# DiligentGraphics/DiligentFX

Measured on AMD Instinct MI355X. Metric: Mpixels/s full PBR+postFX chain @4K; %HBM roofline; 1/2/4/8-GPU scaling, higher is better.
Workload: dtype f32; 1 GPU; full chain PBR+SSR+SSAO+composite+TAA+Bloom+ToneMap 3840x2160 per GPU (BASELINE configs[3]); width=3840, height_per_gpu=2160, storage=fp32 planes, taa=bicubic, ssao=GTAO full-res, ssr=full-res rays, tonemap=Uncharted2+sRGB, ibl=static maps: the shade's apron copy is made once (mifx_postfx_set_static_ibl), fusion_mask=31

## Files before the change

### diligentfx_amd/csrc/api_bloom_taa.cpp

```cpp
#include <cmath>

#include "mifx_objects.h"

using namespace mifx;

mifx_bloom::~mifx_bloom()
{
    for (auto* p : down) delete p;
    for (auto* p : up) delete p;
}

static uint32_t compute_mip_levels_count(uint32_t w, uint32_t h)
{
    uint32_t m = w > h ? w : h, n = 0;
    while (m > 0) { ++n; m >>= 1; }
    return n;
}

extern "C" {

mifx_status mifx_bloom_create(mifx_postfx* ctx, mifx_bloom** out)
{
    MIFX_REQUIRE(ctx != nullptr && out != nullptr, "mifx_bloom_create: null argument");
    *out        = new mifx_bloom();
// ... 59 lines not shown
    p.taa = rows_finer(p.compute0, 4, H);
    const int last = mipCount - 1;
    for (int i = G > 0 ? G : 1; i <= last; ++i) p.up[i] = rows_coarser(p.up[i - 1], 3, int(up[i]->h));
    if (G == 0) p.up[0] = rows_coarser(need, 3, int(up[0]->h));
    p.down[last] = p.up[last];
    for (int i = last - 1; i > G; --i) p.down[i] = rows_hull(p.up[i], rows_finer(p.down[i + 1], 4, int(down[i]->h)));
    return p;
}

mifx_status mifx_bloom::run(const mifx_bloom_render_attribs* ra, int phase, const FusedToneMap* tone_map, const Request& req)
{
    MIFX_RANGE("Bloom");
    mifx_postfx* c = ra->postfx ? ra->postfx : ctx;
    Img  color;
    bool packed = false;
    MIFX_CHECK(to_img_hdr(ra->color, "color", color, packed));
    MIFX_REQUIRE(uint32_t(color.w) == w && uint32_t(color.h) == h, "mifx_bloom_execute: color is %dx%d, the effect was prepared for %ux%u", color.w, color.h, w, h);
    const mifx_bloom_attribs& a = *ra->attribs;
    const int mipCount = mip_count(a);
    MIFX_REQUIRE(mipCount >= 2 && mipCount <= int(down.size()),
                 "mifx_bloom_execute: Radius %g gives %d pyramid levels; the reference reads an unwritten texture below 2 levels", a.Radius, mipCount);
    MIFX_HIP_CHECK(hipSetDevice(c->device));
    hipStream_t s = c->stream;
    const Rows need = c->needed_rows(int(h));
    const Plan p    = make_plan(c->band, need, mipCount, req.halo_level0);
    MIFX_REQUIRE(phase == 0 || p.G >= 0, "mifx_bloom_execute: phased execution needs a row band (mifx_chain_set_row_band)");
    MIFX_REQUIRE(phase != 0 || p.G < 0, "mifx_bloom_execute: a row band is set; run the two phases around the gather of down[%d]", p.G);
    auto dwin = [&](int i) { return p.G >= 0 ? win(down[i]->view(), p.down[i]) : down[i]->view(); };
    auto uwin = [&](int i) { return p.G >= 0 ? win(up[i]->view(), p.up[i]) : up[i]->view(); };
    const int last = mipCount - 1;
    int first = mipCount;
    for (int i = 1; i < mipCount; ++i)
        if (down[i]->w * down[i]->h <= kTailTexels) { first = i; break; }
    bool tail = p.G < 0 && fuse_tail && last >= first + 1 && last - first + 2 <= 8;
    Img  tailDown[8], tailUp[8];
    if (tail)
    {
        for (int i = first - 1; i <= last; ++i) { tailDown[i - first + 1] = down[i]->view(); tailUp[i - first + 1] = up[i]->view(); }
        tail = bloom_tail_fits(tailDown, last - first + 2);
    }
    const int  wide = tail ? first : mipCount;
    if (phase != 2)
    {
        {
            MifxKernelTimer timer(c, "bloom_prefilter_kernel");
            MIFX_CHECK(launch_bloom_prefilter(s, color, p.G >= 0 ? win(down[0]->view(), p.compute0) : down[0]->view(), a, packed));
        }
        if (p.G >= 0 && req.after_level0) MIFX_CHECK(req.after_level0(*down[0], s));
        for (int i = 1; i < wide && (p.G < 0 || i <= p.G); ++i) MIFX_CHECK(launch_bloom_downsample(s, down[i - 1]->view(), dwin(i)));
        if (phase == 1) return MIFX_OK;
    }
    if (p.G >= 0)
        for (int i = p.G + 1; i < wide; ++i) MIFX_CHECK(launch_bloom_downsample(s, down[i - 1]->view(), dwin(i)));
    if (tail) MIFX_CHECK(launch_bloom_tail(s, tailDown, tailUp, last - first + 2));
    for (int i = tail ? first : last; i > 0; --i)
        MIFX_CHECK(launch_bloom_upsample(s, down[i - 1]->view(), i != last ? up[i]->view() : down[i]->view(), uwin(i - 1), a, false));
    if (tone_map)
    {
        MIFX_REQUIRE(tone_map->attribs->iToneMappingMode >= 0 && tone_map->attribs->iToneMappingMode <= MIFX_TONE_MAPPING_MODE_COMMERCE, "unknown tone mapping mode %d",
                     tone_map->attribs->iToneMappingMode);
        MIFX_REQUIRE((tone_map->flags & ~uint32_t(MIFX_TONEMAP_FLAG_CONVERT_OUTPUT_TO_SRGB)) == 0, "unknown tone map flags 0x%x", tone_map->flags);
        Img ldr;
        MIFX_CHECK(to_img_wh(tone_map->ldr, MIFX_FORMAT_F32X4, w, h, "ldr_out", ldr));
        MifxKernelTimer timer(c, "bloom_upsample_tonemap_kernel");
        MIFX_CHECK(launch_bloom_final_tonemap(s, color, up[0]->view(), win(output.view(), need), ldr, a, *tone_map->attribs, tone_map->ave_log_lum, tone_map->flags, !tone_map->skip_output, packed));
        output_deferred  = tone_map->skip_output;
        deferred_color   = color;
        deferred_packed  = packed;
        deferred_attribs = a;
        deferred_rows    = need;
    }
    else
    {
        MifxKernelTimer timer(c, "bloom_upsample_kernel");
        MIFX_CHECK(launch_bloom_upsample(s, color, up[0]->view(), win(output.view(), need), a, true, packed));
        output_deferred = false;
    }
    return MIFX_OK;
}

mifx_status mifx_bloom::run_deferred_output()
{
    if (!output_deferred) return MIFX_OK;
    MIFX_HIP_CHECK(hipSetDevice(ctx->device));
    ctx->queued_outside_execute();
    MIFX_CHECK(launch_bloom_upsample(ctx->stream, deferred_color, up[0]->view(), win(output.view(), deferred_rows), deferred_attribs, true, deferred_packed));
    output_deferred = false;
    return MIFX_OK;
}

mifx_status mifx_bloom_execute(mifx_bloom* fx, const mifx_bloom_render_attribs* ra)
{
    MIFX_REQUIRE(fx != nullptr && ra != nullptr && ra->attribs != nullptr, "mifx_bloom_execute: null argument");
    if (!fx->prepared)
    {
        set_error("mifx_bloom_execute: mifx_bloom_prepare must be called first");
        return MIFX_ERR_INVALID_OP;
    }
    return fx->run(ra, 0, nullptr, mifx_bloom::Request{});
}

mifx_status mifx_bloom_get_output(mifx_bloom* fx, mifx_image2d* out)
{
    MIFX_REQUIRE(fx != nullptr && out != nullptr, "mifx_bloom_get_output: null argument");
    if (!fx->prepared)
    {
        set_error("mifx_bloom_get_output: resources are not prepared");
        return MIFX_ERR_INVALID_OP;
    }
    MIFX_CHECK(fx->run_deferred_output());
    *out = fx->output.desc();
    return MIFX_OK;
}

mifx_status mifx_debug_bloom_set_tail(mifx_bloom* fx, int32_t enable)
{
    MIFX_REQUIRE(fx != nullptr, "mifx_debug_bloom_set_tail: null argument");
    fx->fuse_tail = enable != 0;
    return MIFX_OK;
}

mifx_status mifx_bloom_get_intermediate(mifx_bloom* fx, const char* name, mifx_image2d* out)
{
    MIFX_REQUIRE(fx != nullptr && name != nullptr && out != nullptr, "mifx_bloom_get_intermediate: null argument");
    int k = -1;
    const Plane* p = nullptr;
    if (fx->prepared && std::sscanf(name, "down%d", &k) == 1 && k >= 0 && k < int(fx->down.size())) p = fx->down[k];
    else if (fx->prepared && std::sscanf(name, "up%d", &k) == 1 && k >= 0 && k < int(fx->up.size())) p = fx->up[k];
    MIFX_REQUIRE(p != nullptr, "mifx_bloom_get_intermediate: unknown plane '%s'", name);
    *out = p->desc();
    return MIFX_OK;
}

mifx_status mifx_taa_create(mifx_postfx* ctx, mifx_taa** out)
{
    MIFX_REQUIRE(ctx != nullptr && out != nullptr, "mifx_taa_create: null argument");
    *out        = new mifx_taa();
    (*out)->ctx = ctx;
    return MIFX_OK;
}
void mifx_taa_destroy(mifx_taa* fx) { delete fx; }

mifx_status mifx_taa_prepare(mifx_taa* fx, mifx_postfx* ctx, uint32_t feature_flags)
{
    MIFX_REQUIRE(fx != nullptr && ctx != nullptr, "mifx_taa_prepare: null argument");
    if (!ctx->prepared)
    {
        set_error("mifx_taa_prepare: mifx_postfx_prepare must be called first");
        return MIFX_ERR_INVALID_OP;
    }
    MIFX_REQUIRE((feature_flags & ~7u) == 0, "mifx_taa_prepare: unknown feature flags 0x%x", feature_flags);
// ... 124 lines not shown
```

### diligentfx_amd/csrc/bloom.hip

```cpp
#include "mifx_host.h"
#include "mifx_tonemap.h"

namespace mifx
{
template <int TW, int TH, bool BORDER, class TAG = v4, class LT = v4> struct Tile
{
    static constexpr bool kZeroOutside = BORDER;
    LT* lds;
    Img im;
    int x0, y0;
    static constexpr bool border = BORDER;

#ifndef MIFX_BLOOM_FILL_ROLLED
    template <int NT = 256> MIFX_D void fill() const
    {
        constexpr int N = (TW * TH + NT - 1) / NT;
        const int tid = threadIdx.y * blockDim.x + threadIdx.x;
        v4 v[N];
#pragma unroll
        for (int k = 0; k < N; ++k)
        {
            const int i  = tid + k * NT, ii = i < TW * TH ? i : tid % (TW * TH);
            const int gx = x0 + ii % TW, gy = y0 + ii / TW;
            const v4  t  = ld<TAG>(im, clampi(gx, 0, im.w - 1), clampi(gy, 0, im.h - 1));
            v[k] = t;
        }
#pragma unroll
        for (int k = 0; k < N; ++k) keep_here(v[k]);
#pragma unroll
        for (int k = 0; k < N; ++k)
        {
            const int i  = tid + k * NT;
            const int gx = x0 + i % TW, gy = y0 + i / TW;
            if (i < TW * TH) lds[i] = to_lds((!border || (gx >= 0 && gy >= 0 && gx < im.w && gy < im.h)) ? v[k] : mk4(0.0f), static_cast<const LT*>(nullptr));
// ... 48 lines not shown
        const int x = x0 + (t & 1), y = y0 + (t >> 1);
        if (SRC::kZeroOutside || (x >= 0 && y >= 0 && x < w && y < h))
        {
            MIFX_FMA_BLOCK
            const v4 c = src.fetch(x, y);
            acc = v3{acc.x + c.x * wgt[t], acc.y + c.y * wgt[t], acc.z + c.z * wgt[t]};
        }
    }
    return acc;
}
template <class SRC> MIFX_D v3 sample_linear_clamp_rgb(const SRC& src, int w, int h, float u, float v)
{
    const Bilinear b = bilinear_uc(u * float(w), v * float(h), w, h);
    const v4 t00 = src.fetch(b.x0, b.y0), t10 = src.fetch(b.x1, b.y0), t01 = src.fetch(b.x0, b.y1), t11 = src.fetch(b.x1, b.y1);
    {
        MIFX_FMA_BLOCK
        return v3{t00.x * b.w00 + t10.x * b.w10 + t01.x * b.w01 + t11.x * b.w11, t00.y * b.w00 + t10.y * b.w10 + t01.y * b.w01 + t11.y * b.w11,
                  t00.z * b.w00 + t10.z * b.w10 + t01.z * b.w01 + t11.z * b.w11};
    }
}

struct Taps13 { v3 A, B, C, D, E, F, G, H, I, J, K, L, M; };
template <class SRC> MIFX_D Taps13 fetch13(const SRC& src, int w, int h, v2 uv)
{
    const v2 ts{fdiv(1.0f, float(w)), fdiv(1.0f, float(h))};
    auto S = [&](float ox, float oy) { v3 r = sample_linear_border_rgb(src, w, h, uv.x + ts.x * ox, uv.y + ts.y * oy); MIFX_TAP_FENCE(r); return r; };
    Taps13 t;
    t.A = S(-2.0f, +2.0f); t.B = S(+0.0f, +2.0f); t.C = S(+2.0f, +2.0f);
    t.D = S(-2.0f, +0.0f); t.E = S(+0.0f, +0.0f); t.F = S(+2.0f, +0.0f);
    t.G = S(-2.0f, -2.0f); t.H = S(+0.0f, -2.0f); t.I = S(+2.0f, -2.0f);
    t.J = S(-1.0f, +1.0f); t.K = S(+1.0f, +1.0f); t.L = S(-1.0f, -1.0f); t.M = S(+1.0f, -1.0f);
    return t;
}
MIFX_D v2 pixel_uv(int x, int y, int w, int h)
{
    const v2 ndc{2.0f * fdiv(float(x) + 0.5f, float(w)) - 1.0f, 1.0f - 2.0f * fdiv(float(y) + 0.5f, float(h))};
    return ndc_to_uv(ndc);
}

constexpr int kBX = 32, kBY = 8;
constexpr int kDownTW = 72, kDownTH = 24;
constexpr int kUpTW = 24, kUpTH = 12;
MIFX_HD int tile_origin(int b0, int srcN, int outN, float reach) { return int(floorf((float(b0) + 0.5f) * float(srcN) / float(outN) - 0.5f - reach)) - 1; }
inline bool tile_fits(int srcN, int outN, int blockN, float reach, int tileN)
{
    return float(blockN - 1) * float(srcN) / float(outN) + 2.0f * reach + 5.0f <= float(tileN);
}

typedef v3 UpLds;
typedef v3 DownLds;
template <bool STAGED, class SRC> __global__ __launch_bounds__(256) void bloom_prefilter_kernel(Img in, Img out, float threshold, float softThreshold)
{
    __shared__ DownLds lds[STAGED ? kDownTW * kDownTH : 1];
    const int by0 = int(block_row<4>()) * kBY + out.y0;
    const int x = blockIdx.x * kBX + threadIdx.x, y = by0 + int(threadIdx.y);
    Taps13 t;
    if (STAGED)
    {
        const Tile<kDownTW, kDownTH, true, SRC, DownLds> tile{lds, in, tile_origin(blockIdx.x * kBX, in.w, out.w, 2.0f), tile_origin(by0, in.h, out.h, 2.0f)};
        tile.fill();
        __syncthreads();
        if (x >= out.w || y >= row_end(out)) return;
        t = fetch13(tile, in.w, in.h, pixel_uv(x, y, out.w, out.h));
    }
    else
    {
        if (x >= out.w || y >= row_end(out)) return;
        t = fetch13(Direct<SRC>{in}, in.w, in.h, pixel_uv(x, y, out.w, out.h));
    }
    const float weights[5] = {0.125f, 0.125f, 0.125f, 0.125f, 0.5f};
    const v3 groups[5] = {(t.A + t.B + t.D + t.E) / 4.0f, (t.B + t.C + t.E + t.F) / 4.0f, (t.D + t.E + t.G + t.H) / 4.0f, (t.E + t.F + t.H + t.I) / 4.0f,
                          (t.J + t.K + t.L + t.M) / 4.0f};
    v4 sum = mk4(0.0f);
#pragma unroll
    for (int g = 0; g < 5; ++g)
    {
        const float w = weights[g] * fdiv(1.0f, 1.0f + luminance601(groups[g]));
        sum += mk4(groups[g], 1.0f) * w;
    }
    const v3 color = xyz(sum) / (sum.w + 1.0e-5f);
// ... 3 lines not shown
    soft = clampf(soft, 0.0f, 2.0f * knee);
    soft = fdiv(soft * soft * 0.25f, knee + 1.0e-5f);
    float contribution = fmaxf(soft, brightness - threshold);
    contribution = fdiv(contribution, fmaxf(brightness, 1.0e-5f));
    st<bloom_t>(out, x, y, mk4(color * contribution, 0.0f));
}

template <bool STAGED> __global__ __launch_bounds__(256) void bloom_downsample_kernel(Img in, Img out)
{
    __shared__ DownLds lds[STAGED ? kDownTW * kDownTH : 1];
    const int by0 = int(blockIdx.y) * kBY + out.y0;
    const int x = blockIdx.x * kBX + threadIdx.x, y = by0 + int(threadIdx.y);
    Taps13 t;
    if (STAGED)
    {
        const Tile<kDownTW, kDownTH, true, bloom_t, DownLds> tile{lds, in, tile_origin(blockIdx.x * kBX, in.w, out.w, 2.0f), tile_origin(by0, in.h, out.h, 2.0f)};
        tile.fill();
        __syncthreads();
        if (x >= out.w || y >= row_end(out)) return;
        t = fetch13(tile, in.w, in.h, pixel_uv(x, y, out.w, out.h));
    }
    else
    {
        if (x >= out.w || y >= row_end(out)) return;
        t = fetch13(Direct<bloom_t>{in}, in.w, in.h, pixel_uv(x, y, out.w, out.h));
    }
    v3 c = mk3(0.0f);
    c += (t.A + t.C + t.G + t.I) * 0.03125f;
    c += (t.B + t.D + t.F + t.H) * 0.0625f;
    c += (t.E + t.J + t.K + t.L + t.M) * 0.125f;
    st<bloom_t>(out, x, y, mk4(c, 0.0f));
}

struct TentAxis
{
    int   i[4];
    float w[4];
    bool  regular;
};
MIFX_D TentAxis tent_axis(float u, float ts, int n)
{
    const float l0 = (u + ts * -1.0f) * float(n) - 0.5f, l1 = (u + ts * 0.0f) * float(n) - 0.5f, l2 = (u + ts * 1.0f) * float(n) - 0.5f;
    const float f0 = floorf(l0), f1 = floorf(l1), f2 = floorf(l2);
    const float x0 = l0 - f0, x1 = l1 - f1, x2 = l2 - f2;
    TentAxis a;
    a.regular = (f1 == f0 + 1.0f) && (f2 == f0 + 2.0f);
    const int b = int(f0);
#pragma unroll
    for (int s = 0; s < 4; ++s) a.i[s] = clampi(b + s, 0, n - 1);
    a.w[0] = 0.25f * (1.0f - x0);
    a.w[1] = 0.25f * x0 + 0.5f * (1.0f - x1);
    a.w[2] = 0.5f * x1 + 0.25f * (1.0f - x2);
    a.w[3] = 0.25f * x2;
    return a;
}
template <bool FINAL, bool STAGED> MIFX_D bool bloom_upsample_texel(UpLds* lds, Img input, Img down, Img out, float intensity, float alphaInterp, int srcPacked, int& x, int& y, v4& result)
{
    const int by0 = int(blockIdx.y) * kBY + out.y0;
    x = blockIdx.x * kBX + threadIdx.x;
    y = by0 + int(threadIdx.y);
    const Tile<kUpTW, kUpTH, false, bloom_t, UpLds> tile{lds, down, tile_origin(blockIdx.x * kBX, down.w, out.w, 1.0f), tile_origin(by0, down.h, out.h, 1.0f)};
    if (STAGED)
    {
        tile.fill();
        __syncthreads();
    }
    if (x >= out.w || y >= row_end(out)) return false;
    const v2 uv = pixel_uv(x, y, out.w, out.h);
    const v2 ts{fdiv(1.0f, float(down.w)), fdiv(1.0f, float(down.h))};
    auto S = [&](float ox, float oy) {
        v3 r = STAGED ? sample_linear_clamp_rgb(tile, down.w, down.h, uv.x + ts.x * ox, uv.y + ts.y * oy)
                            : sample_linear_clamp_rgb(Direct<bloom_t>{down}, down.w, down.h, uv.x + ts.x * ox, uv.y + ts.y * oy);
        MIFX_TAP_FENCE(r);
        return r;
    };
    v3 sum;
    const TentAxis ax = tent_axis(uv.x, ts.x, down.w), ay = tent_axis(uv.y, ts.y, down.h);
    if (STAGED && ax.regular && ay.regular)
    {
        sum = mk3(0.0f);
#pragma unroll
        for (int j = 0; j < 4; ++j)
        {
            v3 row = mk3(0.0f);
#pragma unroll
            for (int i = 0; i < 4; ++i)
            {
                MIFX_FMA_BLOCK
// ... 18 lines not shown
    }
    const v4 src4 = FINAL ? ld_hdr_once(input, x, y, srcPacked) : ld<bloom_t>(input, x, y);
    const v3 src  = xyz(src4);
    result = FINAL ? bloom_output_value(mk4(lerp3(src, src + intensity * sum, alphaInterp), src4.w))
                   : mk4(src + sum, 0.0f);
    return true;
}
template <bool FINAL, bool STAGED> __global__ __launch_bounds__(256) void bloom_upsample_kernel(Img input, Img down, Img out, float intensity, float alphaInterp, int srcPacked)
{
    __shared__ UpLds lds[STAGED ? kUpTW * kUpTH : 1];
    int x, y;
    v4  r;
    if (bloom_upsample_texel<FINAL, STAGED>(lds, input, down, out, intensity, alphaInterp, srcPacked, x, y, r))
    {
        st<bloom_t>(out, x, y, r);
    }
}
template <bool STAGED, int MODE, bool SRGB>
__global__ __launch_bounds__(256) void bloom_final_tonemap_kernel(Img input, Img down, Img out, Img ldr, float intensity, float alphaInterp, ToneMapK tm, int writeOut, int srcPacked)
{
    __shared__ UpLds lds[STAGED ? kUpTW * kUpTH : 1];
    int x, y;
    v4  r;
    if (!bloom_upsample_texel<true, STAGED>(lds, input, down, out, intensity, alphaInterp, srcPacked, x, y, r)) return;
    if (writeOut) st<bloom_t>(out, x, y, r);
    r = quantize_v4(r);
    v3 t = tone_map<MODE>(xyz(r), tm);
    if (SRGB) t = linear_to_srgb(t);
    st_v4_late<1>(ldr, x, y, mk4(t, r.w));
}

struct BloomTail
{
    Img      down[8], up[8];
    int      levels;
    unsigned foldMask;
};
struct LdsLevel
{
    static constexpr bool kZeroOutside = false;
    const v4* p;
    int       w, h;
    MIFX_D v4 fetch(int x, int y) const { return p[y * w + x]; }
};
template <class SRC> MIFX_D v3 bloom_upsample_sum(const SRC& src, int dw, int dh, int outW, int outH, int x, int y, bool mayFold)
{
    struct { int w, h; } down{dw, dh};
    const v2 uv = pixel_uv(x, y, outW, outH);
    const v2 ts{fdiv(1.0f, float(down.w)), fdiv(1.0f, float(down.h))};
    const TentAxis ax = tent_axis(uv.x, ts.x, down.w), ay = tent_axis(uv.y, ts.y, down.h);
    v3 sum;
    if (mayFold && ax.regular && ay.regular)
    {
        sum = mk3(0.0f);
#pragma unroll
        for (int j = 0; j < 4; ++j)
        {
            v3 row = mk3(0.0f);
#pragma unroll
            for (int i = 0; i < 4; ++i)
            {
                MIFX_FMA_BLOCK
                const v4 t = src.fetch(ax.i[i], ay.i[j]);
                row = v3{row.x + t.x * ax.w[i], row.y + t.y * ax.w[i], row.z + t.z * ax.w[i]};
            }
            {
                MIFX_FMA_BLOCK
                sum = v3{sum.x + row.x * ay.w[j], sum.y + row.y * ay.w[j], sum.z + row.z * ay.w[j]};
            }
            MIFX_TAP_FENCE(sum);
        }
    }
    else
    {
        auto S = [&](float ox, float oy) { v3 r = sample_linear_clamp_rgb(src, down.w, down.h, uv.x + ts.x * ox, uv.y + ts.y * oy); MIFX_TAP_FENCE(r); return r; };
        const v3 A = S(-1.0f, +1.0f), B = S(+0.0f, +1.0f), C = S(+1.0f, +1.0f);
        const v3 D = S(-1.0f, +0.0f), E = S(+0.0f, +0.0f), F = S(+1.0f, +0.0f);
        const v3 G = S(-1.0f, -1.0f), H = S(+0.0f, -1.0f), I = S(+1.0f, -1.0f);
        sum = E * 0.25f;
        sum += (B + D + F + H) * 0.125f;
        sum += (A + C + G + I) * 0.0625f;
    }
    return sum;
}
constexpr int kTailLdsTexels = 2048 + 2048 / 3 + 64;
__global__ __launch_bounds__(1024) void bloom_tail_kernel(BloomTail t)
{
    __shared__ v4 lds[kTailLdsTexels];
    __shared__ int off[9];
    const int tid = int(threadIdx.x), nthreads = int(blockDim.x);
    if (tid == 0)
    {
        int o = 0;
        for (int l = 1; l < t.levels; ++l) { off[l] = o; o += t.down[l].w * t.down[l].h; }
        off[t.levels] = o;
    }
    __syncthreads();
    for (int l = 1; l < t.levels; ++l)
    {
        const Img in = t.down[l - 1], out = t.down[l];
        v4* dst = lds + off[l];
        for (int i = tid; i < out.w * out.h; i += nthreads)
        {
            const int x = i % out.w, y = i / out.w;
            const v2  uv = pixel_uv(x, y, out.w, out.h);
            const Taps13 s = l == 1 ? fetch13(Direct<bloom_t>{in}, in.w, in.h, uv) : fetch13(LdsLevel{lds + off[l - 1], in.w, in.h}, in.w, in.h, uv);
            v3 c = mk3(0.0f);
            c += (s.A + s.C + s.G + s.I) * 0.03125f;
            c += (s.B + s.D + s.F + s.H) * 0.0625f;
            c += (s.E + s.J + s.K + s.L + s.M) * 0.125f;
            dst[i] = quantize_bloom(mk4(c, 0.0f));
            st<bloom_t>(out, x, y, mk4(c, 0.0f));
        }
        __syncthreads();
    }
    for (int l = t.levels - 1; l >= 2; --l)
    {
        const Img srcImg = t.down[l], out = t.up[l - 1];
        const LdsLevel src{lds + off[l], srcImg.w, srcImg.h};
        v4* acc = lds + off[l - 1];
        const bool mayFold = ((t.foldMask >> (l - 1)) & 1u) != 0u;
        for (int i = tid; i < out.w * out.h; i += nthreads)
// ... 11 lines not shown
static const dim3 kBlock(64, 4, 1);
static const dim3 kBloomBlock(kBX, kBY, 1);
static inline dim3 bloom_grid(const Img& out) { return dim3((out.w + kBX - 1) / kBX, (window_rows(out) + kBY - 1) / kBY, 1); }

mifx_status launch_bloom_prefilter(hipStream_t s, Img in, Img out, const mifx_bloom_attribs& a, bool packedInput)
{
    const bool staged = tile_fits(in.w, out.w, kBX, 2.0f, kDownTW) && tile_fits(in.h, out.h, kBY, 2.0f, kDownTH);
#define MIFX_B1(S, T) hipLaunchKernelGGL((bloom_prefilter_kernel<S, T>), bloom_grid(out), kBloomBlock, 0, s, in, out, a.Threshold, a.SoftTreshold)
    if (packedInput) { if (staged) MIFX_B1(true, bloom_t); else MIFX_B1(false, bloom_t); }
    else { if (staged) MIFX_B1(true, v4); else MIFX_B1(false, v4); }
#undef MIFX_B1
    MIFX_HIP_CHECK(hipGetLastError());
    return MIFX_OK;
}
mifx_status launch_bloom_downsample(hipStream_t s, Img in, Img out)
{
    if (tile_fits(in.w, out.w, kBX, 2.0f, kDownTW) && tile_fits(in.h, out.h, kBY, 2.0f, kDownTH))
        hipLaunchKernelGGL((bloom_downsample_kernel<true>), bloom_grid(out), kBloomBlock, 0, s, in, out);
    else
        hipLaunchKernelGGL((bloom_downsample_kernel<false>), bloom_grid(out), kBloomBlock, 0, s, in, out);
    MIFX_HIP_CHECK(hipGetLastError());
    return MIFX_OK;
}
mifx_status launch_bloom_upsample(hipStream_t s, Img input, Img down, Img out, const mifx_bloom_attribs& a, bool final_pass, bool packedInput)
{
    const bool staged = tile_fits(down.w, out.w, kBX, 1.0f, kUpTW) && tile_fits(down.h, out.h, kBY, 1.0f, kUpTH);
#define MIFX_UP(F, S) hipLaunchKernelGGL((bloom_upsample_kernel<F, S>), bloom_grid(out), kBloomBlock, 0, s, input, down, out, a.Intensity, a.AlphaInterpolation, packedInput ? 1 : 0)
    if (final_pass) { if (staged) MIFX_UP(true, true); else MIFX_UP(true, false); }
    else { if (staged) MIFX_UP(false, true); else MIFX_UP(false, false); }
#undef MIFX_UP
    MIFX_HIP_CHECK(hipGetLastError());
    return MIFX_OK;
}
bool bloom_tail_fits(const Img* down, int count)
{
    int texels = 0;
    for (int i = 1; i < count; ++i) texels += down[i].w * down[i].h;
    return count >= 2 && count <= 8 && texels <= kTailLdsTexels;
}
mifx_status launch_bloom_tail(hipStream_t s, const Img* down, const Img* up, int count)
{
    if (count < 2 || count > 8) { set_error("launch_bloom_tail: %d levels", count); return MIFX_ERR_INVALID_ARG; }
    {
        int texels = 0;
        for (int i = 1; i < count; ++i) texels += down[i].w * down[i].h;
        if (texels > kTailLdsTexels) { set_error("launch_bloom_tail: %d texels exceed the LDS budget of %d", texels, kTailLdsTexels); return MIFX_ERR_INVALID_ARG; }
    }
    BloomTail t{};
    t.levels = count;
    for (int i = 0; i < count; ++i) { t.down[i] = down[i]; t.up[i] = up[i]; }
    for (int l = count - 1; l >= 2; --l)
    {
        const Img& src = t.down[l];
        const Img& out = t.up[l - 1];
        if (tile_fits(src.w, out.w, kBX, 1.0f, kUpTW) && tile_fits(src.h, out.h, kBY, 1.0f, kUpTH)) t.foldMask |= 1u << (l - 1);
    }
    hipLaunchKernelGGL(bloom_tail_kernel, dim3(1, 1, 1), dim3(1024, 1, 1), 0, s, t);
    MIFX_HIP_CHECK(hipGetLastError());
    return MIFX_OK;
}
mifx_status launch_bloom_final_tonemap(hipStream_t s, Img input, Img down, Img out, Img ldr, const mifx_bloom_attribs& a, const mifx_tone_mapping_attribs& attr, float ave_log_lum,
                                       uint32_t flags, bool writeBloomOutput, bool packedInput)
{
    const bool staged = tile_fits(down.w, out.w, kBX, 1.0f, kUpTW) && tile_fits(down.h, out.h, kBY, 1.0f, kUpTH);
    const bool srgb   = (flags & MIFX_TONEMAP_FLAG_CONVERT_OUTPUT_TO_SRGB) != 0;
    const ToneMapK tm = make_tonemapk(attr, ave_log_lum);
#define MIFX_FT(S, M, G) hipLaunchKernelGGL((bloom_final_tonemap_kernel<S, M, G>), bloom_grid(out), kBloomBlock, 0, s, input, down, out, ldr, a.Intensity, a.AlphaInterpolation, tm, writeBloomOutput ? 1 : 0, packedInput ? 1 : 0)
#define MIFX_FT_MODE(M)                                                     \
    if (staged) { if (srgb) MIFX_FT(true, M, true); else MIFX_FT(true, M, false); }    \
    else { if (srgb) MIFX_FT(false, M, true); else MIFX_FT(false, M, false); }
    MIFX_TONEMAP_DISPATCH(attr.iToneMappingMode, MIFX_FT_MODE)
#undef MIFX_FT_MODE
#undef MIFX_FT
    MIFX_HIP_CHECK(hipGetLastError());
    return MIFX_OK;
}
}
```

### diligentfx_amd/csrc/mifx_objects.h

```cpp
#pragma once
#include "mifx_rows.h"
#include <cmath>
#include <functional>
#include <map>
#include <string>
#include <vector>
#include "mifx_host.h"

struct mifx_postfx
{
    int         device = 0;
    hipStream_t stream = nullptr;

    mifx_frame_desc frame{};
    uint32_t        flags    = 0;
    bool            prepared = false;
    bool            executed = false;

    void*       sobol_dev      = nullptr;
    void*       scrambling_dev = nullptr;
    mifx::Plane noise_xy, noise_zw;
    uint32_t    noise_frame = ~0u;

    mifx::Plane  reproj_depth, closest_motion;
    mifx_image2d prev_depth{};
    bool        depth16 = false;
    mifx::Plane prev_depth16;
    mifx_camera_attribs curr_cam{}, prev_cam{};

    mifx::Rows need{0, 0}, prep_rows{0, 0}, band{0, 0};
    int        max_motion = 0;
    mifx::Rows needed_rows(int h) const { return need.empty() ? mifx::Rows{0, h} : mifx::rows_clip(need, h); }

    uint64_t stream_epoch = 0;
    std::vector<hipEvent_t> pending_joins;
    void queued_outside_execute()
    {
        ++stream_epoch;
        for (hipEvent_t e : pending_joins) (void)hipStreamWaitEvent(stream, e, 0);
        pending_joins.clear();
// ... 119 lines not shown
    bool                clean_tiles      = true;
    mifx::Plane res_radiance, res_variance, res_depth;
    mifx::Plane hist_radiance[2], hist_variance[2];
    mifx::Plane output;
    bool               cleanup_pending = false;
    mifx::SsrCleanupIn cleanup_in{};
    mifx::Img          cleanup_normal{};
    mifx::CamK         cleanup_cam{};
    mifx::Rows         cleanup_rows{0, 0};
    mifx_status        run_cleanup();
};

struct mifx_taa
{
    mifx_postfx* ctx = nullptr;
    uint32_t     w = 0, h = 0, flags = 0;
    bool         prepared = false;
    uint32_t     last_frame = ~0u, curr_frame = 0;
    mifx::Plane  accum[2];
    uint32_t     techniques_created = 0;
    bool         technique_ready    = false;
    mifx_status run(const mifx_taa_render_attribs* ra, const mifx::TaaFusedComposite* fused);
};

struct mifx_bloom
{
    mifx_postfx* ctx = nullptr;
    uint32_t     w = 0, h = 0, flags = 0;
    bool         prepared = false;
    std::vector<mifx::Plane*> down, up;
    mifx::Plane  output;
    ~mifx_bloom();
    static constexpr int kGatherLevel = 1;
    static constexpr uint32_t kTailTexels = 512;
    bool fuse_tail = true;
    struct Plan
    {
        int        G = -1;
        mifx::Rows taa{0, 0};
        mifx::Rows own{0, 0};
        mifx::Rows down[16], up[16];
        mifx::Rows compute0{0, 0};
        mifx::Rows own0{0, 0};
    };
    struct Request
    {
        bool halo_level0 = false;
        std::function<mifx_status(const mifx::Plane& level0, hipStream_t s)> after_level0;
    };
    Plan make_plan(mifx::Rows band, mifx::Rows need, int mipCount, bool halo_level0) const;
    int  mip_count(const mifx_bloom_attribs& a) const;
    struct FusedToneMap
    {
        const mifx_image2d*              ldr;
        const mifx_tone_mapping_attribs* attribs;
        float                            ave_log_lum;
        uint32_t                         flags;
        bool                             skip_output = false;
    };
    bool               output_deferred = false;
    mifx::Img          deferred_color{};
    bool               deferred_packed = false;
    mifx_bloom_attribs deferred_attribs{};
    mifx::Rows         deferred_rows{0, 0};
    mifx_status        run_deferred_output();
    mifx_status run(const mifx_bloom_render_attribs* ra, int phase, const FusedToneMap* tone_map, const Request& req);
};

// ... 188 lines not shown
```

### include/mifx.h

```cpp
#ifndef MIFX_H
#define MIFX_H

#include <stdint.h>

#ifdef __cplusplus
extern "C" {
#endif

#define MIFX_API __attribute__((visibility("default")))

typedef int32_t mifx_status;
enum
{
    MIFX_OK                  = 0,
    MIFX_NO_HISTORY          = 1,
    MIFX_ERR_INVALID_ARG     = -1,
    MIFX_ERR_INVALID_OP      = -2,
    MIFX_ERR_HIP             = -3,
    MIFX_ERR_OUT_OF_MEMORY   = -4,
    MIFX_ERR_NOT_IMPLEMENTED = -5,
    MIFX_ERR_COMM            = -6
};
MIFX_API const char* mifx_status_string(mifx_status s);
MIFX_API const char* mifx_last_error(void);
// ... 293 lines not shown
    MIFX_TAA_FEATURE_FLAG_GAUSSIAN_WEIGHTING = 1 << 0,
    MIFX_TAA_FEATURE_FLAG_BICUBIC_FILTER     = 1 << 1,
    MIFX_TAA_FEATURE_FLAG_YCOCG_COLOR_SPACE  = 1 << 2
};
typedef struct mifx_taa_render_attribs
{
    mifx_postfx*            postfx;
    const mifx_image2d*     color;
    const mifx_taa_attribs* attribs;
} mifx_taa_render_attribs;
MIFX_API mifx_status mifx_taa_create(mifx_postfx* ctx, mifx_taa** out);
MIFX_API void        mifx_taa_destroy(mifx_taa* fx);
MIFX_API mifx_status mifx_taa_prepare(mifx_taa* fx, mifx_postfx* ctx, uint32_t feature_flags);
MIFX_API mifx_status mifx_taa_execute(mifx_taa* fx, const mifx_taa_render_attribs* attribs);
MIFX_API mifx_status mifx_taa_get_output(mifx_taa* fx, int32_t is_prev_frame, mifx_image2d* out);
MIFX_API mifx_status mifx_taa_reset_history(mifx_taa* fx);
MIFX_API mifx_status mifx_taa_export_history(mifx_taa* fx, const mifx_image2d* out_color, uint32_t* out_frame_index);
MIFX_API mifx_status mifx_taa_import_history(mifx_taa* fx, const mifx_image2d* color, uint32_t frame_index);
MIFX_API mifx_status mifx_taa_get_jitter_offset(uint32_t frame_index, uint32_t width, uint32_t height, float out_jitter[2]);
MIFX_API mifx_status mifx_taa_get_jittered_proj_matrix(const float proj[16], const float jitter[2], float out_proj[16]);

typedef struct mifx_bloom mifx_bloom;
typedef struct mifx_bloom_render_attribs
{
    mifx_postfx*              postfx;
    const mifx_image2d*       color;
    const mifx_bloom_attribs* attribs;
} mifx_bloom_render_attribs;
MIFX_API mifx_status mifx_bloom_create(mifx_postfx* ctx, mifx_bloom** out);
MIFX_API void        mifx_bloom_destroy(mifx_bloom* fx);
MIFX_API mifx_status mifx_bloom_prepare(mifx_bloom* fx, mifx_postfx* ctx, uint32_t feature_flags);
MIFX_API mifx_status mifx_bloom_execute(mifx_bloom* fx, const mifx_bloom_render_attribs* attribs);
MIFX_API mifx_status mifx_bloom_get_output(mifx_bloom* fx, mifx_image2d* out);
MIFX_API mifx_status mifx_debug_bloom_set_tail(mifx_bloom* fx, int32_t enable);
MIFX_API mifx_status mifx_bloom_get_intermediate(mifx_bloom* fx, const char* name, mifx_image2d* out);

typedef struct mifx_dof mifx_dof;
enum
{
    MIFX_DOF_FEATURE_FLAG_NONE                      = 0u,
    MIFX_DOF_FEATURE_FLAG_ENABLE_TEMPORAL_SMOOTHING = 1u << 0,
    MIFX_DOF_FEATURE_FLAG_ENABLE_KARIS_INVERSE      = 1u << 1
};
typedef struct mifx_dof_render_attribs
{
    mifx_postfx*            postfx;
    const mifx_image2d*     color;
    const mifx_image2d*     depth;
    const mifx_dof_attribs* attribs;
} mifx_dof_render_attribs;
MIFX_API mifx_status mifx_dof_create(mifx_postfx* ctx, mifx_dof** out);
MIFX_API void        mifx_dof_destroy(mifx_dof* fx);
MIFX_API mifx_status mifx_dof_prepare(mifx_dof* fx, mifx_postfx* ctx, uint32_t feature_flags);
MIFX_API mifx_status mifx_dof_execute(mifx_dof* fx, const mifx_dof_render_attribs* attribs);
MIFX_API mifx_status mifx_dof_get_output(mifx_dof* fx, mifx_image2d* out);
MIFX_API mifx_status mifx_dof_get_intermediate(mifx_dof* fx, const char* name, mifx_image2d* out);
MIFX_API mifx_status mifx_dof_reset_history(mifx_dof* fx);
MIFX_API mifx_status mifx_debug_dof_set_last_pass(mifx_dof* fx, uint32_t last_pass);
MIFX_API mifx_status mifx_dof_generate_kernel_points(int32_t ring_count, int32_t ring_density, float* out, uint32_t capacity_points, uint32_t* out_count);

typedef struct mifx_gbuffer
{
    const mifx_image2d* base_color;
    const mifx_image2d* normal;
    const mifx_image2d* material;
    const mifx_image2d* depth;
    const mifx_image2d* emissive;
// ... 464 lines not shown
```

Before: 5482 Mpixels/s.

## Fuse adjacent bloom pyramid levels into paired downsample and upsample kernels

Adds two-level bloom kernels: a paired downsample keeps the intermediate level in LDS and computes two mip levels per launch, and a paired upsample does the same for the upsample chain. The tail plan is extended to cover the whole pyramid from level 1 by default (tail_mode=1), so mid-size levels take fewer launches. It also adds launch counting and a debug query. The aim is to cut kernel launch overhead and global round trips for the small bloom levels. In exchange, apron regions are recomputed redundantly and large-LDS 1024-thread blocks can reduce occupancy.

```diff
diff --git a/diligentfx_amd/csrc/api_bloom_taa.cpp b/diligentfx_amd/csrc/api_bloom_taa.cpp
--- a/diligentfx_amd/csrc/api_bloom_taa.cpp
+++ b/diligentfx_amd/csrc/api_bloom_taa.cpp
@@ -115,29 +115,38 @@
     int first = mipCount;
     for (int i = 1; i < mipCount; ++i)
         if (down[i]->w * down[i]->h <= kTailTexels) { first = i; break; }
-    bool tail = p.G < 0 && fuse_tail && last >= first + 1 && last - first + 2 <= 8;
-    Img  tailDown[8], tailUp[8];
-    if (tail)
-    {
-        for (int i = first - 1; i <= last; ++i) { tailDown[i - first + 1] = down[i]->view(); tailUp[i - first + 1] = up[i]->view(); }
-        tail = bloom_tail_fits(tailDown, last - first + 2);
-    }
+    Img  tailDown[kBloomMaxLevels], tailUp[kBloomMaxLevels];
+    auto range_fits = [&](int f) {
+        if (f < 1 || last - f + 2 > kBloomMaxLevels) return false;
+        for (int i = f - 1; i <= last; ++i) { tailDown[i - f + 1] = down[i]->view(); tailUp[i - f + 1] = up[i]->view(); }
+        return bloom_tail_fits(tailDown, last - f + 2);
+    };
+    bool tail = false;
+    if (p.G < 0 && tail_mode == 1 && range_fits(1)) { tail = true; first = 1; }
+    else if (p.G < 0 && tail_mode != 0 && last >= first + 1) tail = range_fits(first);
     const int  wide = tail ? first : mipCount;
+    if (phase != 2) last_launches = 0;
     if (phase != 2)
     {
         {
             MifxKernelTimer timer(c, "bloom_prefilter_kernel");
             MIFX_CHECK(launch_bloom_prefilter(s, color, p.G >= 0 ? win(down[0]->view(), p.compute0) : down[0]->view(), a, packed));
+            ++last_launches;
         }
         if (p.G >= 0 && req.after_level0) MIFX_CHECK(req.after_level0(*down[0], s));
-        for (int i = 1; i < wide && (p.G < 0 || i <= p.G); ++i) MIFX_CHECK(launch_bloom_downsample(s, down[i - 1]->view(), dwin(i)));
+        for (int i = 1; i < wide && (p.G < 0 || i <= p.G); ++i, ++last_launches) MIFX_CHECK(launch_bloom_downsample(s, down[i - 1]->view(), dwin(i)));
         if (phase == 1) return MIFX_OK;
     }
     if (p.G >= 0)
-        for (int i = p.G + 1; i < wide; ++i) MIFX_CHECK(launch_bloom_downsample(s, down[i - 1]->view(), dwin(i)));
-    if (tail) MIFX_CHECK(launch_bloom_tail(s, tailDown, tailUp, last - first + 2));
-    for (int i = tail ? first : last; i > 0; --i)
+        for (int i = p.G + 1; i < wide; ++i, ++last_launches) MIFX_CHECK(launch_bloom_downsample(s, down[i - 1]->view(), dwin(i)));
+    if (tail)
+    {
+        MIFX_CHECK(launch_bloom_tail(s, tailDown, tailUp, last - first + 2));
+        last_launches += bloom_tail_plan(tailDown, last - first + 2).launches;
+    }
+    for (int i = tail ? first : last; i > 0; --i, ++last_launches)
         MIFX_CHECK(launch_bloom_upsample(s, down[i - 1]->view(), i != last ? up[i]->view() : down[i]->view(), uwin(i - 1), a, false));
+    ++last_launches;
     if (tone_map)
     {
         MIFX_REQUIRE(tone_map->attribs->iToneMappingMode >= 0 && tone_map->attribs->iToneMappingMode <= MIFX_TONE_MAPPING_MODE_COMMERCE, "unknown tone mapping mode %d",
@@ -196,10 +205,18 @@
     return MIFX_OK;
 }
 
-mifx_status mifx_debug_bloom_set_tail(mifx_bloom* fx, int32_t enable)
+mifx_status mifx_debug_bloom_set_tail(mifx_bloom* fx, int32_t mode)
 {
     MIFX_REQUIRE(fx != nullptr, "mifx_debug_bloom_set_tail: null argument");
-    fx->fuse_tail = enable != 0;
+    MIFX_REQUIRE(mode >= 0 && mode <= 2, "mifx_debug_bloom_set_tail: mode %d (0: per-level launches, 1: pairs and tail, 2: tail only)", mode);
+    fx->tail_mode = mode;
+    return MIFX_OK;
+}
+
+mifx_status mifx_debug_bloom_get_launches(mifx_bloom* fx, int32_t* launches)
+{
+    MIFX_REQUIRE(fx != nullptr && launches != nullptr, "mifx_debug_bloom_get_launches: null argument");
+    *launches = fx->last_launches;
     return MIFX_OK;
 }
 
diff --git a/diligentfx_amd/csrc/bloom.hip b/diligentfx_amd/csrc/bloom.hip
--- a/diligentfx_amd/csrc/bloom.hip
+++ b/diligentfx_amd/csrc/bloom.hip
@@ -1,5 +1,6 @@
 #include "mifx_host.h"
 #include "mifx_tonemap.h"
+#include "mifx_bloom_pairs.h"
 
 namespace mifx
 {
@@ -114,20 +115,7 @@
     t.J = S(-1.0f, +1.0f); t.K = S(+1.0f, +1.0f); t.L = S(-1.0f, -1.0f); t.M = S(+1.0f, -1.0f);
     return t;
 }
-MIFX_D v2 pixel_uv(int x, int y, int w, int h)
-{
-    const v2 ndc{2.0f * fdiv(float(x) + 0.5f, float(w)) - 1.0f, 1.0f - 2.0f * fdiv(float(y) + 0.5f, float(h))};
-    return ndc_to_uv(ndc);
-}
-
-constexpr int kBX = 32, kBY = 8;
-constexpr int kDownTW = 72, kDownTH = 24;
-constexpr int kUpTW = 24, kUpTH = 12;
-MIFX_HD int tile_origin(int b0, int srcN, int outN, float reach) { return int(floorf((float(b0) + 0.5f) * float(srcN) / float(outN) - 0.5f - reach)) - 1; }
-inline bool tile_fits(int srcN, int outN, int blockN, float reach, int tileN)
-{
-    return float(blockN - 1) * float(srcN) / float(outN) + 2.0f * reach + 5.0f <= float(tileN);
-}
+
 
 typedef v3 UpLds;
 typedef v3 DownLds;
@@ -197,28 +185,6 @@
     st<bloom_t>(out, x, y, mk4(c, 0.0f));
 }
 
-struct TentAxis
-{
-    int   i[4];
-    float w[4];
-    bool  regular;
-};
-MIFX_D TentAxis tent_axis(float u, float ts, int n)
-{
-    const float l0 = (u + ts * -1.0f) * float(n) - 0.5f, l1 = (u + ts * 0.0f) * float(n) - 0.5f, l2 = (u + ts * 1.0f) * float(n) - 0.5f;
-    const float f0 = floorf(l0), f1 = floorf(l1), f2 = floorf(l2);
-    const float x0 = l0 - f0, x1 = l1 - f1, x2 = l2 - f2;
-    TentAxis a;
-    a.regular = (f1 == f0 + 1.0f) && (f2 == f0 + 2.0f);
-    const int b = int(f0);
-#pragma unroll
-    for (int s = 0; s < 4; ++s) a.i[s] = clampi(b + s, 0, n - 1);
-    a.w[0] = 0.25f * (1.0f - x0);
-    a.w[1] = 0.25f * x0 + 0.5f * (1.0f - x1);
-    a.w[2] = 0.5f * x1 + 0.25f * (1.0f - x2);
-    a.w[3] = 0.25f * x2;
-    return a;
-}
 template <bool FINAL, bool STAGED> MIFX_D bool bloom_upsample_texel(UpLds* lds, Img input, Img down, Img out, float intensity, float alphaInterp, int srcPacked, int& x, int& y, v4& result)
 {
     const int by0 = int(blockIdx.y) * kBY + out.y0;
@@ -303,7 +269,7 @@
 
 struct BloomTail
 {
-    Img      down[8], up[8];
+    Img      down[kBloomMaxLevels], up[kBloomMaxLevels];
     int      levels;
     unsigned foldMask;
 };
@@ -354,11 +320,82 @@
     }
     return sum;
 }
-constexpr int kTailLdsTexels = 2048 + 2048 / 3 + 64;
+
+template <int TW, bool BORDER> struct MidTile
+{
+    static constexpr bool kZeroOutside = BORDER;
+    const v3* p;
+    int       x0, y0;
+    MIFX_D v4 fetch(int x, int y) const { return mk4(p[(y - y0) * TW + (x - x0)], 0.0f); }
+};
+MIFX_D v3 bloom_downsample_sum(const Taps13& t)
+{
+    v3 c = mk3(0.0f);
+    c += (t.A + t.C + t.G + t.I) * 0.03125f;
+    c += (t.B + t.D + t.F + t.H) * 0.0625f;
+    c += (t.E + t.J + t.K + t.L + t.M) * 0.125f;
+    return c;
+}
+constexpr int kDown2Threads = 1024;
+__global__ __launch_bounds__(kDown2Threads) void bloom_downsample2_kernel(Img src, Img mid, Img out)
+{
+    __shared__ DownLds ldsSrc[kDown2SrcTW * kDown2SrcTH];
+    __shared__ DownLds ldsMid[kDown2MidTW * kDown2MidTH];
+    const PairAxis ax = down2_axis_x(int(blockIdx.x), src.w, mid.w, out.w), ay = down2_axis_y(int(blockIdx.y), src.h, mid.h, out.h);
+    const Tile<kDown2SrcTW, kDown2SrcTH, true, bloom_t, DownLds> tile{ldsSrc, src, ax.src0, ay.src0};
+    tile.fill<kDown2Threads>();
+    __syncthreads();
+    const int tid = int(threadIdx.x);
+    for (int i = tid; i < kDown2MidTW * kDown2MidTH; i += kDown2Threads)
+    {
+        const int x = ax.mid0 + i % kDown2MidTW, y = ay.mid0 + i / kDown2MidTW;
+        v3 stored = mk3(0.0f);
+        if (x >= ax.lo && x < ax.hi && y >= ay.lo && y < ay.hi)
+        {
+            const v4 c = mk4(bloom_downsample_sum(fetch13(tile, src.w, src.h, pixel_uv(x, y, mid.w, mid.h))), 0.0f);
+            stored = xyz(quantize_bloom(c));
+            if (x >= ax.own0 && x < ax.own1 && y >= ay.own0 && y < ay.own1) st<bloom_t>(mid, x, y, c);
+        }
+        ldsMid[i] = stored;
+    }
+    __syncthreads();
+    const int x = int(blockIdx.x) * kDown2BX + tid % kDown2BX, y = int(blockIdx.y) * kDown2BY + tid / kDown2BX;
+    if (tid >= kDown2BX * kDown2BY || x >= out.w || y >= out.h) return;
+    const MidTile<kDown2MidTW, true> m{ldsMid, ax.mid0, ay.mid0};
+    st<bloom_t>(out, x, y, mk4(bloom_downsample_sum(fetch13(m, mid.w, mid.h, pixel_uv(x, y, out.w, out.h))), 0.0f));
+}
+__global__ __launch_bounds__(256) void bloom_upsample2_kernel(Img src, Img downMid, Img upMid, Img downOut, Img upOut, int foldMid, int foldOut)
+{
+    __shared__ UpLds ldsSrc[kUp2SrcTW * kUp2SrcTH];
+    __shared__ UpLds ldsMid[kUp2MidTW * kUp2MidTH];
+    const PairAxis ax = up2_axis_x(int(blockIdx.x), src.w, upMid.w, upOut.w), ay = up2_axis_y(int(blockIdx.y), src.h, upMid.h, upOut.h);
+    const Tile<kUp2SrcTW, kUp2SrcTH, false, bloom_t, UpLds> tile{ldsSrc, src, ax.src0, ay.src0};
+    tile.fill();
+    __syncthreads();
+    const int tid = int(threadIdx.y) * kBX + int(threadIdx.x);
+    {
+        const int x = ax.mid0 + tid % kUp2MidTW, y = ay.mid0 + tid / kUp2MidTW;
+        if (tid < kUp2MidTW * kUp2MidTH && x >= ax.lo && x < ax.hi && y >= ay.lo && y < ay.hi)
+        {
+            const v3 sum = bloom_upsample_sum(tile, src.w, src.h, upMid.w, upMid.h, x, y, foldMid != 0);
+            const v4 r   = mk4(xyz(ld<bloom_t>(downMid, x, y)) + sum, 0.0f);
+            ldsMid[tid]  = xyz(quantize_bloom(r));
+            if (x >= ax.own0 && x < ax.own1 && y >= ay.own0 && y < ay.own1) st<bloom_t>(upMid, x, y, r);
+        }
+    }
+    __syncthreads();
+    const int x = int(blockIdx.x) * kBX + int(threadIdx.x), y = int(blockIdx.y) * kBY + int(threadIdx.y);
+    if (x >= upOut.w || y >= upOut.h) return;
+    const MidTile<kUp2MidTW, false> m{ldsMid, ax.mid0, ay.mid0};
+    const v3 sum = bloom_upsample_sum(m, upMid.w, upMid.h, upOut.w, upOut.h, x, y, foldOut != 0);
+    st<bloom_t>(upOut, x, y, mk4(xyz(ld<bloom_t>(downOut, x, y)) + sum, 0.0f));
+}
+
+constexpr int kTailLdsTexels = kBloomTailLdsTexels;
 __global__ __launch_bounds__(1024) void bloom_tail_kernel(BloomTail t)
 {
     __shared__ v4 lds[kTailLdsTexels];
-    __shared__ int off[9];
+    __shared__ int off[kBloomMaxLevels + 1];
     const int tid = int(threadIdx.x), nthreads = int(blockDim.x);
     if (tid == 0)
     {
@@ -436,31 +473,55 @@
     MIFX_HIP_CHECK(hipGetLastError());
     return MIFX_OK;
 }
+static inline bool up_staged(const Img& src, const Img& out)
+{
+    return tile_fits(src.w, out.w, kBX, 1.0f, kUpTW) && tile_fits(src.h, out.h, kBY, 1.0f, kUpTH);
+}
 bool bloom_tail_fits(const Img* down, int count)
 {
-    int texels = 0;
-    for (int i = 1; i < count; ++i) texels += down[i].w * down[i].h;
-    return count >= 2 && count <= 8 && texels <= kTailLdsTexels;
+    return bloom_tail_plan(down, count).fused;
 }
 mifx_status launch_bloom_tail(hipStream_t s, const Img* down, const Img* up, int count)
 {
-    if (count < 2 || count > 8) { set_error("launch_bloom_tail: %d levels", count); return MIFX_ERR_INVALID_ARG; }
-    {
-        int texels = 0;
-        for (int i = 1; i < count; ++i) texels += down[i].w * down[i].h;
-        if (texels > kTailLdsTexels) { set_error("launch_bloom_tail: %d texels exceed the LDS budget of %d", texels, kTailLdsTexels); return MIFX_ERR_INVALID_ARG; }
-    }
-    BloomTail t{};
-    t.levels = count;
-    for (int i = 0; i < count; ++i) { t.down[i] = down[i]; t.up[i] = up[i]; }
-    for (int l = count - 1; l >= 2; --l)
-    {
-        const Img& src = t.down[l];
-        const Img& out = t.up[l - 1];
-        if (tile_fits(src.w, out.w, kBX, 1.0f, kUpTW) && tile_fits(src.h, out.h, kBY, 1.0f, kUpTH)) t.foldMask |= 1u << (l - 1);
-    }
-    hipLaunchKernelGGL(bloom_tail_kernel, dim3(1, 1, 1), dim3(1024, 1, 1), 0, s, t);
-    MIFX_HIP_CHECK(hipGetLastError());
+    if (count < 2 || count > kBloomMaxLevels) { set_error("launch_bloom_tail: %d levels", count); return MIFX_ERR_INVALID_ARG; }
+    const BloomTailPlan plan = bloom_tail_plan(down, count);
+    const int wideEnd = plan.tail < count ? plan.tail : count;
+    for (int i = 1; i < wideEnd; ++i)
+    {
+        if ((plan.downPair >> i) & 1u)
+        {
+            const Img& out = down[i + 1];
+            hipLaunchKernelGGL(bloom_downsample2_kernel, dim3((out.w + kDown2BX - 1) / kDown2BX, (out.h + kDown2BY - 1) / kDown2BY, 1), dim3(kDown2Threads, 1, 1), 0, s, down[i - 1], down[i], out);
+            MIFX_HIP_CHECK(hipGetLastError());
+            ++i;
+        }
+        else MIFX_CHECK(launch_bloom_downsample(s, down[i - 1], down[i]));
+    }
+    if (plan.tail < count)
+    {
+        const int n = count - plan.tail + 1;
+        BloomTail t{};
+        t.levels = n;
+        for (int i = 0; i < n; ++i) { t.down[i] = down[plan.tail - 1 + i]; t.up[i] = up[plan.tail - 1 + i]; }
+        for (int l = n - 1; l >= 2; --l)
+            if (up_staged(t.down[l], t.up[l - 1])) t.foldMask |= 1u << (l - 1);
+        hipLaunchKernelGGL(bloom_tail_kernel, dim3(1, 1, 1), dim3(1024, 1, 1), 0, s, t);
+        MIFX_HIP_CHECK(hipGetLastError());
+    }
+    const mifx_bloom_attribs unused{};
+    auto source = [&](int j) { return j == count - 1 ? down[j] : up[j]; };
+    for (int j = wideEnd - 1 - (plan.tail < count ? 0 : 1); j >= 1; --j)
+    {
+        if ((plan.upPair >> j) & 1u)
+        {
+            const Img& out = up[j - 1];
+            hipLaunchKernelGGL(bloom_upsample2_kernel, bloom_grid(out), kBloomBlock, 0, s, source(j + 1), down[j], up[j], down[j - 1], out, up_staged(down[j + 1], up[j]) ? 1 : 0,
+                               up_staged(up[j], out) ? 1 : 0);
+            MIFX_HIP_CHECK(hipGetLastError());
+            --j;
+        }
+        else MIFX_CHECK(launch_bloom_upsample(s, down[j], source(j + 1), up[j], unused, false));
+    }
     return MIFX_OK;
 }
 mifx_status launch_bloom_final_tonemap(hipStream_t s, Img input, Img down, Img out, Img ldr, const mifx_bloom_attribs& a, const mifx_tone_mapping_attribs& attr, float ave_log_lum,
diff --git a/diligentfx_amd/csrc/mifx_bloom_pairs.h b/diligentfx_amd/csrc/mifx_bloom_pairs.h
--- /dev/null
+++ b/diligentfx_amd/csrc/mifx_bloom_pairs.h
@@ -0,0 +1,132 @@
+#pragma once
+#include "mifx_device.h"
+
+namespace mifx
+{
+MIFX_HD v2 pixel_uv(int x, int y, int w, int h)
+{
+    const v2 ndc{2.0f * fdiv(float(x) + 0.5f, float(w)) - 1.0f, 1.0f - 2.0f * fdiv(float(y) + 0.5f, float(h))};
+    return ndc_to_uv(ndc);
+}
+
+struct TentAxis
+{
+    int   i[4];
+    float w[4];
+    bool  regular;
+};
+MIFX_HD TentAxis tent_axis(float u, float ts, int n)
+{
+    const float l0 = (u + ts * -1.0f) * float(n) - 0.5f, l1 = (u + ts * 0.0f) * float(n) - 0.5f, l2 = (u + ts * 1.0f) * float(n) - 0.5f;
+    const float f0 = floorf(l0), f1 = floorf(l1), f2 = floorf(l2);
+    const float x0 = l0 - f0, x1 = l1 - f1, x2 = l2 - f2;
+    TentAxis a;
+    a.regular = (f1 == f0 + 1.0f) && (f2 == f0 + 2.0f);
+    const int b = int(f0);
+#pragma unroll
+    for (int s = 0; s < 4; ++s) a.i[s] = clampi(b + s, 0, n - 1);
+    a.w[0] = 0.25f * (1.0f - x0);
+    a.w[1] = 0.25f * x0 + 0.5f * (1.0f - x1);
+    a.w[2] = 0.5f * x1 + 0.25f * (1.0f - x2);
+    a.w[3] = 0.25f * x2;
+    return a;
+}
+
+constexpr int kBX = 32, kBY = 8;
+constexpr int kDownTW = 72, kDownTH = 24;
+constexpr int kUpTW = 24, kUpTH = 12;
+MIFX_HD int tile_origin(int b0, int srcN, int outN, float reach) { return int(floorf((float(b0) + 0.5f) * float(srcN) / float(outN) - 0.5f - reach)) - 1; }
+MIFX_HD bool tile_fits(int srcN, int outN, int blockN, float reach, int tileN)
+{
+    return float(blockN - 1) * float(srcN) / float(outN) + 2.0f * reach + 5.0f <= float(tileN);
+}
+
+struct PairAxis
+{
+    int mid0, lo, hi, src0, own0, own1;
+};
+MIFX_HD PairAxis pair_axis(int b, int blockN, int ownN, int midTileN, int srcN, int midN, int outN, float reach)
+{
+    PairAxis a;
+    a.mid0 = tile_origin(b * blockN, midN, outN, reach);
+    a.lo   = a.mid0 > 0 ? a.mid0 : 0;
+    a.hi   = a.mid0 + midTileN < midN ? a.mid0 + midTileN : midN;
+    a.src0 = tile_origin(a.lo, srcN, midN, reach);
+    const int nb = (outN + blockN - 1) / blockN;
+    a.own0 = b * ownN < midN ? b * ownN : midN;
+    a.own1 = (b + 1 < nb && (b + 1) * ownN < midN) ? (b + 1) * ownN : midN;
+    return a;
+}
+inline bool pair_axis_fits(int blockN, int ownN, int midTileN, int srcTileN, int srcN, int midN, int outN, float reach)
+{
+    if (srcN < 1 || midN < 1 || outN < 1) return false;
+    if (!tile_fits(midN, outN, blockN < outN ? blockN : outN, reach, midTileN)) return false;
+    if (!tile_fits(srcN, midN, midTileN < midN ? midTileN : midN, reach, srcTileN)) return false;
+    const int nb = (outN + blockN - 1) / blockN;
+    for (int b = 0; b < nb; ++b)
+    {
+        const PairAxis a = pair_axis(b, blockN, ownN, midTileN, srcN, midN, outN, reach);
+        if (a.own0 < a.lo || a.own1 > a.hi) return false;
+    }
+    return true;
+}
+constexpr int kDown2BX = 16, kDown2BY = 8, kDown2MidTW = 40, kDown2MidTH = 24, kDown2SrcTW = 88, kDown2SrcTH = 56;
+constexpr int kUp2MidTW = 23, kUp2MidTH = 11, kUp2SrcTW = 18, kUp2SrcTH = 12;
+MIFX_HD PairAxis down2_axis_x(int b, int srcN, int midN, int outN) { return pair_axis(b, kDown2BX, 2 * kDown2BX, kDown2MidTW, srcN, midN, outN, 2.0f); }
+MIFX_HD PairAxis down2_axis_y(int b, int srcN, int midN, int outN) { return pair_axis(b, kDown2BY, 2 * kDown2BY, kDown2MidTH, srcN, midN, outN, 2.0f); }
+MIFX_HD PairAxis up2_axis_x(int b, int srcN, int midN, int outN) { return pair_axis(b, kBX, kBX / 2, kUp2MidTW, srcN, midN, outN, 1.0f); }
+MIFX_HD PairAxis up2_axis_y(int b, int srcN, int midN, int outN) { return pair_axis(b, kBY, kBY / 2, kUp2MidTH, srcN, midN, outN, 1.0f); }
+inline bool down2_fits(int sw, int sh, int mw, int mh, int ow, int oh)
+{
+    return pair_axis_fits(kDown2BX, 2 * kDown2BX, kDown2MidTW, kDown2SrcTW, sw, mw, ow, 2.0f) && pair_axis_fits(kDown2BY, 2 * kDown2BY, kDown2MidTH, kDown2SrcTH, sh, mh, oh, 2.0f);
+}
+inline bool up2_fits(int sw, int sh, int mw, int mh, int ow, int oh)
+{
+    return pair_axis_fits(kBX, kBX / 2, kUp2MidTW, kUp2SrcTW, sw, mw, ow, 1.0f) && pair_axis_fits(kBY, kBY / 2, kUp2MidTH, kUp2SrcTH, sh, mh, oh, 1.0f);
+}
+
+constexpr int kBloomMaxLevels = 16;
+constexpr int kBloomTailTexels = 512;
+constexpr int kBloomTailLdsTexels = 2048 + 2048 / 3 + 64;
+constexpr int kBloomPairTexels = 131072;
+
+struct BloomTailPlan
+{
+    int      tail      = 0;
+    unsigned downPair  = 0;
+    unsigned upPair    = 0;
+    int      launches  = 0;
+    bool     fused     = false;
+};
+inline BloomTailPlan bloom_tail_plan(const Img* down, int count)
+{
+    BloomTailPlan p;
+    p.tail = count;
+    if (count < 2 || count > kBloomMaxLevels) return p;
+    auto texels = [&](int i) { return long(down[i].w) * long(down[i].h); };
+    for (int i = 1; i < count; ++i)
+        if (texels(i) <= kBloomTailTexels) { p.tail = i; break; }
+    if (p.tail < count)
+    {
+        long sum = 0;
+        for (int i = p.tail; i < count; ++i) sum += texels(i);
+        if (count - 1 < p.tail + 1 || sum > kBloomTailLdsTexels) p.tail = count;
+    }
+    const int wideEnd = p.tail < count ? p.tail : count;
+    for (int i = 1; i < wideEnd; ++i, ++p.launches)
+        if (i + 1 < wideEnd && texels(i) <= kBloomPairTexels && down2_fits(down[i - 1].w, down[i - 1].h, down[i].w, down[i].h, down[i + 1].w, down[i + 1].h))
+        {
+            p.downPair |= 1u << i;
+            ++i;
+        }
+    if (p.tail < count) ++p.launches;
+    for (int j = (p.tail < count ? p.tail : count - 1) - 1; j >= 1; --j, ++p.launches)
+        if (j - 1 >= 1 && texels(j) <= kBloomPairTexels && up2_fits(down[j + 1].w, down[j + 1].h, down[j].w, down[j].h, down[j - 1].w, down[j - 1].h))
+        {
+            p.upPair |= 1u << j;
+            --j;
+        }
+    p.fused = p.tail < count || p.downPair != 0u || p.upPair != 0u;
+    return p;
+}
+}
diff --git a/diligentfx_amd/csrc/mifx_objects.h b/diligentfx_amd/csrc/mifx_objects.h
--- a/diligentfx_amd/csrc/mifx_objects.h
+++ b/diligentfx_amd/csrc/mifx_objects.h
@@ -6,6 +6,7 @@
 #include <string>
 #include <vector>
 #include "mifx_host.h"
+#include "mifx_bloom_pairs.h"
 
 struct mifx_postfx
 {
@@ -191,8 +192,10 @@
     mifx::Plane  output;
     ~mifx_bloom();
     static constexpr int kGatherLevel = 1;
-    static constexpr uint32_t kTailTexels = 512;
-    bool fuse_tail = true;
+    static constexpr uint32_t kTailTexels = mifx::kBloomTailTexels;
+    static constexpr uint32_t kPairTexels = mifx::kBloomPairTexels;
+    int tail_mode = 1;
+    int last_launches = 0;
     struct Plan
     {
         int        G = -1;
diff --git a/include/mifx.h b/include/mifx.h
--- a/include/mifx.h
+++ b/include/mifx.h
@@ -349,7 +349,8 @@
 MIFX_API mifx_status mifx_bloom_prepare(mifx_bloom* fx, mifx_postfx* ctx, uint32_t feature_flags);
 MIFX_API mifx_status mifx_bloom_execute(mifx_bloom* fx, const mifx_bloom_render_attribs* attribs);
 MIFX_API mifx_status mifx_bloom_get_output(mifx_bloom* fx, mifx_image2d* out);
-MIFX_API mifx_status mifx_debug_bloom_set_tail(mifx_bloom* fx, int32_t enable);
+MIFX_API mifx_status mifx_debug_bloom_set_tail(mifx_bloom* fx, int32_t mode);
+MIFX_API mifx_status mifx_debug_bloom_get_launches(mifx_bloom* fx, int32_t* launches);
 MIFX_API mifx_status mifx_bloom_get_intermediate(mifx_bloom* fx, const char* name, mifx_image2d* out);
 
 typedef struct mifx_dof mifx_dof;
```

Result: no change. 5507 Mpixels/s (median of 6 runs) (+0.4%).
